# darchr/EmbeddingTables.jl

Measured on AMD Instinct MI355X. Metric: embedding lookups/sec + achieved HBM GB/s (% of roofline), 26 tables x dim128 at B=65536, higher is better.
Workload: dtype f32

## Files before the change

embeddingtables.jl_amd/csrc/et_lookup.hip:

```cpp
#include <type_traits>
#include "et_common.h"
#include "et_lookup_order.h"

#include <stdlib.h>
#include <string.h>

#include <mutex>
#include <utility>
#include <vector>

namespace et {

struct XcdQueue;
struct LookupPack {
    et_lookup_desc d[ET_MAX_TABLES_PER_LAUNCH];
    XcdQueue* queue = nullptr;
};

template <typename T, int D>
struct VecGeom {
    static constexpr int N = 16 / (int)sizeof(T);
    static constexpr int VPR = D / N;
    static constexpr int LPR = VPR < 64 ? VPR : 64;
    static constexpr int NV = VPR / LPR;
// ... 210 lines not shown
    const uint32_t ldt = (uint32_t)d.ld_table, nr = (uint32_t)d.nrows;
    const int vpr = MK ? d.dim / G::N : G::VPR;
    int64_t bag = chunk * per_round * rounds + wave * G::GPW + g;
    long long my_next = load_idx_chunk<G::LPR>(
        d.idx + (bag < batch ? bag : batch - 1) * d.ld_idx, cnt0, sub);
    for (int r = 0; r < rounds; ++r) {
        if (bag >= batch) break;
        const long long my = my_next;
        const int64_t nbag = bag + per_round;
        if (r + 1 < rounds)
            my_next = load_idx_chunk<G::LPR>(
                d.idx + (nbag < batch ? nbag : batch - 1) * d.ld_idx, cnt0, sub);
        bag_sum_vec<T, A, D, U, NT, NTL, PG, MK>(table, ldt, nr, (uint32_t)d.cols_per_page,
                                                 d.idx + bag * d.ld_idx, pool, my,
                                                 dst + bag * ld_dst + d.dst_row_off, g, sub, vpr);
        bag = nbag;
    }
}

typedef const __attribute__((address_space(4))) int64_t* cidx_ptr;

__device__ __forceinline__ cidx_ptr as_scalar_idx(const int64_t* p) {
    return (cidx_ptr)(uintptr_t)p;
}

__device__ __forceinline__ uint64_t row_off_s(int64_t v, uint32_t ldb, uint32_t nrows,
                                              uint32_t& bad) {
    const uint32_t lo = (uint32_t)v - 1u;
    const uint32_t borrow = (uint32_t)(((uint64_t)lo - (uint64_t)nrows) >> 32);
    bad |= (uint32_t)((uint64_t)v >> 32) | ~borrow;
    return (((uint64_t)__umulhi(lo, ldb)) << 32) | (uint64_t)(lo * ldb);
}

template <typename T, typename A, int UU, bool NTL>
__device__ __forceinline__ bool load_add_s(uintptr_t tb, uint32_t ldb, uint32_t nrows,
                                           cidx_ptr ia, cidx_ptr ib, uint64_t hmask,
                                           uint64_t lane_off, bool first_batch,
                                           A (&acc)[16 / sizeof(T)]) {
    constexpr int N = 16 / (int)sizeof(T);
    typedef const __attribute__((address_space(1))) u32x4 gvec;
    uint64_t oa[UU], dd[UU];
    uint32_t bad = 0u;
#pragma unroll
    for (int u = 0; u < UU; ++u) {
        oa[u] = row_off_s(ia[u], ldb, nrows, bad);
        dd[u] = row_off_s(ib[u], ldb, nrows, bad) - oa[u];
    }
    if (bad) return false;
    u32x4 buf[UU];
#pragma unroll
    for (int u = 0; u < UU; ++u) {
        const uint64_t a = ((dd[u] & hmask) + lane_off) + (tb + oa[u]);
        const gvec* src = reinterpret_cast<const gvec*>(a);
        if constexpr (NTL)
            buf[u] = __builtin_nontemporal_load(src);
        else
            buf[u] = *src;
    }
#pragma unroll
    for (int u = 0; u < UU; ++u) {
        T x[N];
        __builtin_memcpy(x, &buf[u], 16);
#pragma unroll
        for (int k = 0; k < N; ++k) {
            if (u == 0)
                acc[k] = first_batch ? A(x[k]) : A(acc[k] + A(x[k]));
            else
                acc[k] = A(acc[k] + A(x[k]));
        }
    }
    return true;
}

template <typename T, typename A>
__device__ __forceinline__ void bag_pair_checked(uintptr_t tb, uint32_t ldb, uint32_t nrows,
                                                 const int64_t* ia, const int64_t* ib, bool hi,
                                                 int sub, int pool, A* acc, int* bad) {
    constexpr int N = 16 / (int)sizeof(T);
    const int64_t* ip = hi ? ib : ia;
#pragma unroll 1
    for (int i = 0; i < pool; ++i) {
        const uint64_t r = (uint64_t)(ip[i] - 1);
        const bool ok = r < (uint64_t)nrows;
        *bad += ok ? 0 : 1;
        const u32x4 v = *(reinterpret_cast<const u32x4*>(
                              tb + (uint64_t)(ok ? (uint32_t)r : 0u) * ldb) + sub);
        T x[N];
        unpack16<T, N>(ok ? v : u32x4{0u, 0u, 0u, 0u}, x);
        for (int k = 0; k < N; ++k) acc[k] = i == 0 ? A(x[k]) : A(acc[k] + A(x[k]));
    }
}

template <typename T, typename A, int U, bool NT, bool NTL>
__device__ __forceinline__ void run_bags_s(const et_lookup_desc& d, int64_t batch,
                                           T* __restrict__ dst, int64_t ld_dst, int64_t chunk,
                                           int rounds) {
    constexpr int N = 16 / (int)sizeof(T);
    const int lane = threadIdx.x & 63;
    const int wave = __builtin_amdgcn_readfirstlane(threadIdx.x >> 6);
    const bool hi = lane >= 32;
    const int sub = lane & 31;
    uint32_t hm = hi ? ~0u : 0u;
    asm volatile("" : "+v"(hm));
    const uint64_t hmask = ((uint64_t)hm << 32) | hm, lane_off = (uint64_t)sub * 16u;
    const uintptr_t tb = reinterpret_cast<uintptr_t>(d.table);
    const uint32_t ldb = (uint32_t)(d.ld_table * (int64_t)sizeof(T)), nr = (uint32_t)d.nrows;
    const int pool = d.pool;
    int64_t bag = chunk * 8 * rounds + 2 * wave;
    for (int r = 0; r < rounds; ++r, bag += 8) {
        if (bag >= batch) break;
        const bool has_b = bag + 1 < batch;
        const cidx_ptr ia = as_scalar_idx(d.idx + bag * d.ld_idx);
        const cidx_ptr ib = has_b ? as_scalar_idx(d.idx + (bag + 1) * d.ld_idx) : ia;
        A acc[N];
#pragma unroll
        for (int k = 0; k < N; ++k) acc[k] = A(0);
        bool ok = true;
        int i0 = 0;
#define ET_LOAD_ADD_S(UU) \
    load_add_s<T, A, UU, NTL>(tb, ldb, nr, ia + i0, ib + i0, hmask, lane_off, i0 == 0, acc)
        for (; ok && i0 + U <= pool; i0 += U) ok = ET_LOAD_ADD_S(U);
        if constexpr (U > 4) {
            if (ok && pool - i0 >= 4) {
                ok = ET_LOAD_ADD_S(4);
                i0 += 4;
            }
        }
        if constexpr (U > 2) {
            if (ok && pool - i0 >= 2) {
                ok = ET_LOAD_ADD_S(2);
                i0 += 2;
            }
        }
        if (ok && pool - i0 >= 1) ok = ET_LOAD_ADD_S(1);
#undef ET_LOAD_ADD_S
        int bad = 0;
        if (!ok)
            bag_pair_checked<T, A>(tb, ldb, nr, d.idx + bag * d.ld_idx,
                                   d.idx + (has_b ? bag + 1 : bag) * d.ld_idx, hi, sub, pool, acc,
                                   &bad);
        if (hi && !has_b) bad = 0;
        if (bad && sub == 0) note_oob(bad);
        if (!hi || has_b) {
            T y[N];
#pragma unroll
            for (int k = 0; k < N; ++k) y[k] = T(acc[k]);
            u32x4* o =
                reinterpret_cast<u32x4*>(dst + (bag + (hi ? 1 : 0)) * ld_dst + d.dst_row_off) + sub;
            store16<NT>(o, pack16<T, N>(y));
        }
    }
}

template <typename T, typename A, int D, int U, bool NT, bool PG = false, bool MK = false,
          bool SG = false>
__global__ __launch_bounds__(256) void k_pooled_vec(LookupPack pack, int ntables, int64_t batch,
                                                    T* __restrict__ dst, int64_t ld_dst,
                                                    int rounds) {
    const int64_t item = blockIdx.x;
    const int t = (int)(item % ntables);
    const int64_t chunk = item / ntables;
    if constexpr (SG)
        run_bags_s<T, A, U, NT, false>(pack.d[t], batch, dst, ld_dst, chunk, rounds);
    else
        run_bags<T, A, D, U, NT, false, PG, MK>(pack.d[t], batch, dst, ld_dst, chunk, rounds);
}

constexpr int kXcds = 8;
static_assert(kXcds == et_order::kXcds && ET_MAX_TABLES_PER_LAUNCH == et_order::kMaxTables,
              "et_lookup_order.h");

constexpr int kMaxStripeEntries = et_order::kMaxEntries;
struct StripeMap {
    uint32_t entry[kXcds][kMaxStripeEntries];
    int nent;
    uint32_t ntload_mask;
    uint32_t prio_mask;
    int nheavy;
    int affinity;
    int fab_share;
    et_order::ClassOrder order[2];
};

template <typename T, typename A, int D, int U, bool NT, bool SG>
__device__ __forceinline__ void striped_body(const LookupPack& pack, const StripeMap& sm,
                                             int ntables, int64_t batch, T* __restrict__ dst,
                                             int64_t ld_dst, int rounds, int64_t stripe_chunks,
                                             int64_t nchunks, int x = blockIdx.x % kXcds,
                                             int64_t slot = blockIdx.x / kXcds) {
    const int k = (int)(slot % ntables);
    const int64_t j = slot / ntables;
    const uint32_t e = sm.entry[x][k];
    const int t = (int)(e & 0xff);
    const int64_t chunk = (int64_t)((e >> 8) & 0xff) * stripe_chunks + j;
    if (j >= stripe_chunks || chunk >= nchunks) return;
    if ((sm.prio_mask >> t) & 1u) __builtin_amdgcn_s_setprio(2);
    if constexpr (SG) {
        if ((sm.ntload_mask >> t) & 1u)
            run_bags_s<T, A, U, NT, true>(pack.d[t], batch, dst, ld_dst, chunk, rounds);
        else
            run_bags_s<T, A, U, NT, false>(pack.d[t], batch, dst, ld_dst, chunk, rounds);
    } else {
        if ((sm.ntload_mask >> t) & 1u)
            run_bags<T, A, D, U, NT, true>(pack.d[t], batch, dst, ld_dst, chunk, rounds);
        else
            run_bags<T, A, D, U, NT, false>(pack.d[t], batch, dst, ld_dst, chunk, rounds);
    }
}

#ifdef ET_WG_TIMELINE
constexpr uint32_t kTlCap = 1u << 17;
__device__ uint4 g_tl[kTlCap][2];
#endif

__device__ __forceinline__ uint64_t tl_begin() {
#ifdef ET_WG_TIMELINE
    return __builtin_amdgcn_s_memrealtime();
#else
    return 0;
#endif
}

__device__ __forceinline__ void tl_stamp(uint64_t t0, const StripeMap& sm, int ntables,
                                         int64_t stripe_chunks, int64_t nchunks, int x,
                                         int64_t slot) {
#ifdef ET_WG_TIMELINE
    __syncthreads();
    if (threadIdx.x == 0 && blockIdx.x < kTlCap) {
        const uint64_t t1 = __builtin_amdgcn_s_memrealtime();
        uint32_t xcc, hw;
        asm volatile("s_getreg_b32 %0, hwreg(HW_REG_XCC_ID)" : "=s"(xcc));
        asm volatile("s_getreg_b32 %0, hwreg(HW_REG_HW_ID)" : "=s"(hw));
        uint32_t t = 0xffu;
        if (x >= 0) {
            const int64_t j = slot / ntables;
            const uint32_t e = sm.entry[x][slot % ntables];
            const int64_t chunk = (int64_t)((e >> 8) & 0xff) * stripe_chunks + j;
            t = (j >= stripe_chunks || chunk >= nchunks ? 0xffu : (e & 0xffu)) | ((uint32_t)x << 8);
        }
        g_tl[blockIdx.x][0] = make_uint4((uint32_t)t0, (uint32_t)(t0 >> 32), (uint32_t)t1,
                                         (uint32_t)(t1 >> 32));
        g_tl[blockIdx.x][1] = make_uint4(t, xcc, hw, gridDim.x);
    }
#endif
}

template <typename T, typename A, int D, int U, bool NT, bool SG = false>
__global__ __launch_bounds__(256) void k_pooled_vec_striped(LookupPack pack, StripeMap sm,
                                                            int ntables, int64_t batch,
                                                            T* __restrict__ dst, int64_t ld_dst,
                                                            int rounds, int64_t stripe_chunks,
                                                            int64_t nchunks) {
    const uint64_t t0 = tl_begin();
    striped_body<T, A, D, U, NT, SG>(pack, sm, ntables, batch, dst, ld_dst, rounds, stripe_chunks,
                                     nchunks);
    tl_stamp(t0, sm, ntables, stripe_chunks, nchunks, blockIdx.x % kXcds, blockIdx.x / kXcds);
}

struct XcdQueue {
    uint32_t head[kXcds][2];
    uint32_t done;
    uint32_t pad[32 - 2 * kXcds - 1];
};
static_assert(sizeof(XcdQueue) == ET_LOOKUP_QUEUE_BYTES, "queue block size (include/embtab.h)");

__device__ __forceinline__ uint32_t cu_hash16(uint32_t hw) {
    const uint32_t cu = (hw >> 8) & 15u, sh = (hw >> 12) & 1u, se = (hw >> 13) & 7u;
    const uint32_t v = (cu + 3u * se + 5u * sh) & 15u;
    return ((v & 1u) << 3) | ((v & 2u) << 1) | ((v & 4u) >> 1) | ((v & 8u) >> 3);
}

__device__ __forceinline__ uint32_t claim_class(XcdQueue& q, const StripeMap& sm, uint32_t x,
                                                uint32_t c, uint32_t nheavy, uint32_t ntables,
                                                uint32_t sc) {
    const uint32_t h = atomicAdd(&q.head[x][c], 1u);
    const uint32_t slot = et_order::class_slot(sm.order[c], x, c, h, nheavy, ntables, sc);
    return slot == et_order::kNone ? ~0u : x * (ntables * sc) + slot;
}

__device__ __forceinline__ uint32_t claim_pref(XcdQueue& q, const StripeMap& sm, uint32_t x0,
                                               uint32_t p, uint32_t nheavy, uint32_t ntables,
                                               uint32_t sc) {
    constexpr uint32_t M = (uint32_t)(kXcds - 1);
    uint32_t it = claim_class(q, sm, x0, p, nheavy, ntables, sc);
    if (it == ~0u && p == 1u) it = claim_class(q, sm, x0, 0u, nheavy, ntables, sc);
    for (uint32_t k = 1; it == ~0u && k < (uint32_t)kXcds; ++k)
        it = claim_class(q, sm, (x0 + k) & M, 0u, nheavy, ntables, sc);
    if (it == ~0u && p == 0u) it = claim_class(q, sm, x0, 1u, nheavy, ntables, sc);
    for (uint32_t k = 1; it == ~0u && k < (uint32_t)kXcds; ++k)
        it = claim_class(q, sm, (x0 + k) & M, 1u, nheavy, ntables, sc);
    return it;
}

template <typename T, typename A, int D, int U, bool NT, bool SG>
__global__ __launch_bounds__(256) void k_pooled_vec_queued(LookupPack pack, StripeMap sm,
                                                           int ntables, int64_t batch,
                                                           T* __restrict__ dst, int64_t ld_dst,
                                                           int rounds, int64_t stripe_chunks,
                                                           int64_t nchunks) {
    const uint64_t t0 = tl_begin();
    __shared__ uint32_t s_item;
    XcdQueue& q = *pack.queue;
    const uint32_t per = (uint32_t)(ntables * stripe_chunks);
    if (threadIdx.x == 0) {
        uint32_t xcc;
        asm volatile("s_getreg_b32 %0, hwreg(HW_REG_XCC_ID)" : "=s"(xcc));
        uint32_t it = ~0u;
        if (sm.affinity != 0) {
            const uint32_t x0 = xcc & (uint32_t)(kXcds - 1);
            const uint32_t nh = (uint32_t)sm.nheavy, sc = (uint32_t)stripe_chunks;
            uint32_t hw;
            asm volatile("s_getreg_b32 %0, hwreg(HW_REG_HW_ID)" : "=s"(hw));
            const uint32_t p = cu_hash16(hw) < (uint32_t)sm.fab_share ? 0u : 1u;
            it = claim_pref(q, sm, x0, p, nh, (uint32_t)ntables, sc);
        } else
        for (uint32_t k = 0; k < (uint32_t)kXcds; ++k) {
            const uint32_t x = (xcc + k) & (uint32_t)(kXcds - 1);
            const uint32_t h = atomicAdd(&q.head[x][0], 1u);
            if (h < per) {
                it = x * per + h;
                break;
            }
        }
        s_item = it;
    }
    __syncthreads();
    const uint32_t it = s_item;
    if (it != ~0u)
        striped_body<T, A, D, U, NT, SG>(pack, sm, ntables, batch, dst, ld_dst, rounds,
                                         stripe_chunks, nchunks, (int)(it / per),
                                         (int64_t)(it % per));
    tl_stamp(t0, sm, ntables, stripe_chunks, nchunks, it != ~0u ? (int)(it / per) : -1,
             (int64_t)(it % per));
    if (threadIdx.x == 0 && atomicAdd(&q.done, 1u) == gridDim.x - 1u) {
        uint32_t* w = reinterpret_cast<uint32_t*>(&q);
        for (int i = 0; i < (int)(sizeof(XcdQueue) / sizeof(uint32_t)); ++i) atomicExch(&w[i], 0u);
    }
}

template <int RB, bool NT>
__global__ __launch_bounds__(256) void k_gather_vec(LookupPack pack, int ntables, int64_t batch,
                                                    char* __restrict__ dst, int64_t ld_dst_b,
                                                    int es, int rounds) {
    constexpr int VPR = RB / 16;
    constexpr int LPR = VPR < 64 ? VPR : 64;
    constexpr int NV = VPR / LPR;
// ... 44 lines not shown
                    store16<NT>(o + v * LPR, okv[u] ? buf[u][v] : u32x4{0u, 0u, 0u, 0u});
            }
        }
        if (bad && sub == 0) note_oob(bad);
    }
}

template <int RB, bool NT, bool NTL, int U, int W = 4>
__global__ __launch_bounds__(64 * W) void k_gather_one(LookupPack pack, int ntables, int64_t batch,
                                                       char* __restrict__ dst, int64_t ld_dst_b,
                                                       int es) {
#ifdef ET_WG_TIMELINE
    const uint64_t tl0 = __builtin_amdgcn_s_memrealtime();
#endif
    constexpr int VPR = RB / 16;
    static_assert(VPR <= 64 && 64 % VPR == 0, "one vector per lane");
    constexpr int GPW = 64 / VPR;
    const int64_t item = blockIdx.x;
    const int t = (int)(item % ntables);
    const int64_t chunk = item / ntables;
    const et_lookup_desc& d = pack.d[t];
    const char* table = reinterpret_cast<const char*>(d.table);
    const int64_t ld_b = d.ld_table * es;
    const int lane = threadIdx.x & 63, wave = threadIdx.x >> 6;
    const int g = lane / VPR, sub = lane % VPR;
    const int64_t per_round = W * GPW;
    const int64_t bag0 = chunk * per_round * U + wave * GPW + g;
    int64_t iv[U];
#pragma unroll
    for (int u = 0; u < U; ++u) {
        int64_t b = bag0 + u * per_round;
        b = b < batch ? b : batch - 1;
        iv[u] = d.idx[b * d.ld_idx];
    }
    u32x4 cur[U];
    bool ok[U];
#pragma unroll
    for (int u = 0; u < U; ++u) {
        const uint64_t row = (uint64_t)(iv[u] - 1);
        ok[u] = row < (uint64_t)d.nrows;
        const u32x4* src = reinterpret_cast<const u32x4*>(table + (ok[u] ? row * (uint64_t)ld_b : 0)) + sub;
        if constexpr (NTL) cur[u] = __builtin_nontemporal_load(src);
        else cur[u] = *src;
    }
#ifdef ET_WG_TIMELINE
    asm volatile("" ::: "memory");
    const uint64_t tl1 = __builtin_amdgcn_s_memrealtime();
#endif
    int bad = 0;
#pragma unroll
    for (int u = 0; u < U; ++u) {
        const int64_t bag = bag0 + u * per_round;
        if (bag < batch) {
            bad += ok[u] ? 0 : 1;
            u32x4* o = reinterpret_cast<u32x4*>(dst + bag * ld_dst_b + d.dst_row_off * es) + sub;
            store16<NT>(o, ok[u] ? cur[u] : u32x4{0u, 0u, 0u, 0u});
        }
    }
    if (bad && sub == 0) note_oob(bad);
#ifdef ET_WG_TIMELINE
    asm volatile("s_waitcnt vmcnt(0)" ::: "memory");
    __syncthreads();
    if (threadIdx.x == 0 && blockIdx.x < kTlCap) {
        const uint64_t tl2 = __builtin_amdgcn_s_memrealtime();
        uint32_t xcc;
        asm volatile("s_getreg_b32 %0, hwreg(HW_REG_XCC_ID)" : "=s"(xcc));
        g_tl[blockIdx.x][0] = make_uint4((uint32_t)tl0, (uint32_t)(tl0 >> 32), (uint32_t)tl1,
                                         (uint32_t)(tl1 >> 32));
        g_tl[blockIdx.x][1] = make_uint4((uint32_t)tl2, (uint32_t)(tl2 >> 32), xcc, gridDim.x);
    }
#endif
}

template <typename O, typename T>
__device__ __forceinline__ O convert_elt(T x) {
    if constexpr ((__is_same(T, __bf16) || __is_same(O, __bf16)) && !__is_same(T, float) &&
                  !__is_same(O, float))
        return O((float)x);
    else
        return O(x);
}

template <typename T, typename A, bool NT, typename O = T>
__global__ __launch_bounds__(256) void k_pooled_generic(LookupPack pack, int ntables,
                                                        int64_t batch, O* __restrict__ dst,
                                                        int64_t ld_dst) {
    constexpr int K = 4;
    const int64_t item = blockIdx.x;
    const int t = (int)(item % ntables);
    const int64_t chunk = item / ntables;
    const et_lookup_desc& d = pack.d[t];
    const T* table = reinterpret_cast<const T*>(d.table);
    const int lane = threadIdx.x & 63, wave = threadIdx.x >> 6;
    const int64_t bag = chunk * 4 + wave;
    if (bag >= batch) return;
    const int64_t* ip = d.idx + bag * d.ld_idx;
    O* out = dst + bag * ld_dst + d.dst_row_off;
    const int dim = d.dim, pool = d.pool;
    for (int f0 = 0; f0 < dim; f0 += 64 * K) {
        A acc[K];
#pragma unroll
        for (int k = 0; k < K; ++k) acc[k] = A(0);
        for (int i = 0; i < pool; ++i) {
            uint64_t row = (uint64_t)(ip[i] - 1);
            const bool ok = row < (uint64_t)d.nrows;
            if (!ok && lane == 0 && f0 == 0) note_oob();
            row = ok ? row : 0;
            const T* src = col_ptr<const T>(d.table, d.ld_table, d.cols_per_page, row);
#pragma unroll
            for (int k = 0; k < K; ++k) {
                const int f = f0 + lane + 64 * k;
                if (f < dim) {
                    const T x = ok ? src[f] : T(0);
                    acc[k] = i == 0 ? A(x) : A(acc[k] + A(x));
                }
            }
        }
#pragma unroll
        for (int k = 0; k < K; ++k) {
            const int f = f0 + lane + 64 * k;
            if (f < dim) store_scalar<NT>(out + f, convert_elt<O>(T(acc[k])));
        }
    }
}


inline bool gather_rb_ok(int64_t rb) {
    return rb == 32 || rb == 64 || rb == 128 || rb == 256 || rb == 512 || rb == 1024 ||
           rb == 2048 || rb == 4096;
}

int max_rounds();

inline int rounds_for(int64_t batch, int64_t bags_per_round, int ntables) {
    int64_t blocks1 = (batch + bags_per_round - 1) / bags_per_round * ntables;
    int rounds = 1;
    const int mr = max_rounds();
    while (rounds < mr && blocks1 / (rounds * 2) >= 4096) rounds *= 2;
    return rounds;
}

struct LookupTuning {
    int striped = 1;
    int queued = 1;
    int ntload = 1;
    int64_t ntload_bytes = 256ll << 20;
    int max_rounds = 8;
    int64_t light_bytes = 4 << 20;
    int sgpr = 1;
    int heavy_prio = 0;
    int affinity = 1;
    int fab_share = 8;
    et_order::Policy order = {1, 3, 1 << 20};
};

inline const LookupTuning& tuning() {
    static LookupTuning t = [] {
        LookupTuning v;
#ifdef ET_EXPERIMENTS
        if (const char* e = getenv("ET_SCHED")) {
            v.striped = strcmp(e, "linear") != 0;
            v.queued = v.striped && strcmp(e, "stripe") != 0;
        }
        v.ntload = (int)ET_KNOB("ET_NTLOAD", v.ntload);
        v.ntload_bytes = ET_KNOB("ET_NTLOAD_BYTES", v.ntload_bytes);
        v.max_rounds = (int)ET_KNOB("ET_ROUNDS", v.max_rounds);
        if (v.max_rounds < 1) v.max_rounds = 1;
        v.light_bytes = ET_KNOB("ET_LIGHT_BYTES", v.light_bytes);
        v.sgpr = (int)ET_KNOB("ET_SGPR", v.sgpr);
        v.heavy_prio = (int)ET_KNOB("ET_HEAVY_PRIO", v.heavy_prio);
        if (const char* e = getenv("ET_AFFINITY")) v.affinity = *e == 'A' ? 1 : 0;
        v.fab_share = (int)ET_KNOB("ET_FAB_SHARE", v.fab_share);
        v.order.cache_major = (int)ET_KNOB("ET_ORDER_CACHE", v.order.cache_major);
        v.order.fab = (int)ET_KNOB("ET_ORDER_FAB", v.order.fab);
        v.order.phase_bytes = ET_KNOB("ET_PHASE_BYTES", v.order.phase_bytes);
#endif
        return v;
    }();
    return t;
}

int max_rounds() { return tuning().max_rounds; }

inline void build_stripe_map(const LookupPack& pack, int n, int es, bool queued, StripeMap& sm) {
    const LookupTuning& tu = tuning();
    int64_t bytes[ET_MAX_TABLES_PER_LAUNCH];
    sm.ntload_mask = 0;
    sm.prio_mask = 0;
    for (int t = 0; t < n; ++t) {
        bytes[t] = pack.d[t].nrows * pack.d[t].ld_table * es;
        if (bytes[t] > tu.light_bytes) {
            if (tu.heavy_prio) sm.prio_mask |= 1u << t;
            if (tu.ntload && bytes[t] > tu.ntload_bytes) sm.ntload_mask |= 1u << t;
        }
    }
    sm.nent = et_order::place_stripes(bytes, n, tu.light_bytes, sm.entry, &sm.nheavy);
    sm.affinity = sm.nheavy > 0 && sm.nheavy < sm.nent ? tu.affinity : 0;
    sm.fab_share = tu.fab_share < 0 ? 0 : tu.fab_share > 16 ? 16 : tu.fab_share;
    if (sm.fab_share == 0) sm.affinity = 0;
    memset(sm.order, 0, sizeof(sm.order));
    if (queued && sm.affinity != 0)
        for (int x = 0; x < kXcds; ++x)
            et_order::order_xcd(sm.entry[x], x, sm.nent, sm.nheavy, bytes, sm.ntload_mask, tu.order,
                                sm.order);
}

template <typename T, typename A, int D, bool NT, bool PG = false, bool MK = false>
int launch_pooled_vec(const LookupPack& pack, int n, int64_t batch, void* dst, int64_t ld_dst,
                      hipStream_t s) {
    using G = VecGeom<T, D>;
    constexpr int U = G::U;
    constexpr bool kSG = !PG && !MK && D * (int)sizeof(T) == 512;
    bool sg = kSG && tuning().sgpr;
    for (int t = 0; t < n && sg; ++t) sg = pack.d[t].ld_table * (int64_t)sizeof(T) < (1ll << 32);
    const int64_t per_round = sg ? 8 : 4 * G::GPW;
    const int rounds = rounds_for(batch, per_round, n);
    const int64_t nchunks = (batch + per_round * rounds - 1) / (per_round * rounds);
    if (nchunks <= 0) return ET_OK;
    const bool striped = !PG && !MK && n > 1 && tuning().striped;
    StripeMap sm;
    int64_t stripe_chunks = 0, grid = nchunks * n;
    const bool queued = striped && pack.queue && tuning().queued;
    if (striped) {
        build_stripe_map(pack, n, (int)sizeof(T), queued, sm);
        stripe_chunks = (nchunks + kXcds - 1) / kXcds;
        grid = (int64_t)kXcds * sm.nent * stripe_chunks;
    }
    if (grid > 0x7fffffffll) return fail(ET_ERR_ARG, "grid too large");
    auto launch = [&](auto loop) -> int {
        constexpr bool SG = decltype(loop)::value;
        T* out = reinterpret_cast<T*>(dst);
        if constexpr (!PG && !MK) {
            if (queued) {
                hipLaunchKernelGGL((k_pooled_vec_queued<T, A, D, U, NT, SG>), dim3((unsigned)grid),
                                   dim3(256), 0, s, pack, sm, sm.nent, batch, out, ld_dst, rounds,
                                   stripe_chunks, nchunks);
                ET_LAUNCH_CHECK("k_pooled_vec_queued");
                return ET_OK;
            }
            if (striped) {
                hipLaunchKernelGGL((k_pooled_vec_striped<T, A, D, U, NT, SG>), dim3((unsigned)grid),
                                   dim3(256), 0, s, pack, sm, sm.nent, batch, out, ld_dst, rounds,
                                   stripe_chunks, nchunks);
                ET_LAUNCH_CHECK("k_pooled_vec_striped");
                return ET_OK;
            }
        }
        hipLaunchKernelGGL((k_pooled_vec<T, A, D, U, NT, PG, MK, SG>), dim3((unsigned)grid),
                           dim3(256), 0, s, pack, n, batch, out, ld_dst, rounds);
        ET_LAUNCH_CHECK("k_pooled_vec");
        return ET_OK;
    };
    if constexpr (kSG) {
        if (sg) return launch(std::true_type{});
    }
    return launch(std::false_type{});
}

template <int RB, bool NT>
int launch_gather_rb(const LookupPack& pack, int n, int64_t batch, void* dst, int64_t ld_dst,
                     int es, hipStream_t s) {
    constexpr int VPR = RB / 16;
    constexpr int LPR = VPR < 64 ? VPR : 64;
    constexpr int NV = VPR / LPR;
    constexpr int U = NV >= 8 ? 1 : 8 / NV;
    const int64_t per_round = 4 * (64 / LPR) * U;
    if constexpr (NV == 1 && U == 8) {
        bool ntl = tuning().ntload != 0;
        for (int t = 0; t < n && ntl; ++t)
            ntl = pack.d[t].nrows * pack.d[t].ld_table * es > tuning().ntload_bytes;
        constexpr int kU = 8, kW = 4;
        const int64_t pw = kW * (64 / LPR) * kU;
        const int64_t g1 = (batch + pw - 1) / pw * n;
        if (g1 <= 0) return ET_OK;
        if (g1 > 0x7fffffffll) return fail(ET_ERR_ARG, "grid too large");
        if (ntl)
            hipLaunchKernelGGL((k_gather_one<RB, NT, true, kU, kW>), dim3((unsigned)g1),
                               dim3(64 * kW), 0, s, pack, n, batch, reinterpret_cast<char*>(dst),
                               ld_dst * es, es);
        else
            hipLaunchKernelGGL((k_gather_one<RB, NT, false, kU, kW>), dim3((unsigned)g1),
                               dim3(64 * kW), 0, s, pack, n, batch, reinterpret_cast<char*>(dst),
                               ld_dst * es, es);
        ET_LAUNCH_CHECK("k_gather_one");
        return ET_OK;
    }
    const int rounds = rounds_for(batch, per_round, n);
    const int64_t nchunks = (batch + per_round * rounds - 1) / (per_round * rounds);
    const int64_t grid = nchunks * n;
    if (grid <= 0) return ET_OK;
    if (grid > 0x7fffffffll) return fail(ET_ERR_ARG, "grid too large");
    hipLaunchKernelGGL((k_gather_vec<RB, NT>), dim3((unsigned)grid), dim3(256), 0, s, pack, n,
                       batch, reinterpret_cast<char*>(dst), ld_dst * es, es, rounds);
    ET_LAUNCH_CHECK("k_gather_vec");
    return ET_OK;
}

template <bool NT>
int launch_gather(const LookupPack& pack, int n, int64_t rb, int64_t batch, void* dst,
                  int64_t ld_dst, int es, hipStream_t s) {
    switch (rb) {
        case 32: return launch_gather_rb<32, NT>(pack, n, batch, dst, ld_dst, es, s);
        case 64: return launch_gather_rb<64, NT>(pack, n, batch, dst, ld_dst, es, s);
        case 128: return launch_gather_rb<128, NT>(pack, n, batch, dst, ld_dst, es, s);
        case 256: return launch_gather_rb<256, NT>(pack, n, batch, dst, ld_dst, es, s);
        case 512: return launch_gather_rb<512, NT>(pack, n, batch, dst, ld_dst, es, s);
        case 1024: return launch_gather_rb<1024, NT>(pack, n, batch, dst, ld_dst, es, s);
        case 2048: return launch_gather_rb<2048, NT>(pack, n, batch, dst, ld_dst, es, s);
        case 4096: return launch_gather_rb<4096, NT>(pack, n, batch, dst, ld_dst, es, s);
    }
    return fail(ET_ERR_UNSUPPORTED, "gather row bytes %lld", (long long)rb);
}

template <typename T, typename A, bool NT, bool PG = false>
int launch_pooled_dim(const LookupPack& pack, int n, int D, int64_t batch, void* dst,
                      int64_t ld_dst, hipStream_t s) {
    switch (D) {
        case 16: return launch_pooled_vec<T, A, 16, NT, PG>(pack, n, batch, dst, ld_dst, s);
        case 32: return launch_pooled_vec<T, A, 32, NT, PG>(pack, n, batch, dst, ld_dst, s);
        case 64: return launch_pooled_vec<T, A, 64, NT, PG>(pack, n, batch, dst, ld_dst, s);
        case 128: return launch_pooled_vec<T, A, 128, NT, PG>(pack, n, batch, dst, ld_dst, s);
        case 256: return launch_pooled_vec<T, A, 256, NT, PG>(pack, n, batch, dst, ld_dst, s);
        case 512: return launch_pooled_vec<T, A, 512, NT, PG>(pack, n, batch, dst, ld_dst, s);
    }
    return fail(ET_ERR_UNSUPPORTED, "vector dim %d", D);
}

template <typename T, typename A, bool NT>
int launch_pooled_masked(const LookupPack& pack, int n, int D, int64_t batch, void* dst,
                         int64_t ld_dst, hipStream_t s) {
#define ET_MK(C)                                                                              \
    case C:                                                                                   \
        if constexpr (C / (16 / (int)sizeof(T)) >= 1)                                         \
            return launch_pooled_vec<T, A, C, NT, false, true>(pack, n, batch, dst, ld_dst,   \
                                                               s);                            \
        break;
    switch (masked_capacity(D)) {
        ET_MK(16)
        ET_MK(32)
        ET_MK(64)
        ET_MK(128)
        ET_MK(256)
        ET_MK(512)
        ET_MK(1024)
        ET_MK(2048)
    }
#undef ET_MK
    return fail(ET_ERR_UNSUPPORTED, "masked vector dim %d", D);
}

template <typename T, typename A, bool NT>
int launch_generic(const LookupPack& pack, int n, int64_t batch, void* dst, int64_t ld_dst,
                   hipStream_t s) {
    const int64_t grid = (batch + 3) / 4 * n;
    if (grid <= 0) return ET_OK;
    if (grid > 0x7fffffffll) return fail(ET_ERR_ARG, "grid too large");
    hipLaunchKernelGGL((k_pooled_generic<T, A, NT>), dim3((unsigned)grid), dim3(256), 0, s, pack,
                       n, batch, reinterpret_cast<T*>(dst), ld_dst);
    ET_LAUNCH_CHECK("k_pooled_generic");
    return ET_OK;
}

enum GroupKind { kGather = 0, kPooledVec = 1, kGeneric = 2, kPagedVec = 3, kMaskedVec = 4 };

template <typename T, typename A, bool NT>
int launch_group_typed(GroupKind kind, const LookupPack& pack, int n, int D, int64_t batch,
                       void* dst, int64_t ld_dst, hipStream_t s) {
    const int es = (int)sizeof(T);
    if (kind == kGather)
        return launch_gather<NT>(pack, n, (int64_t)D * es, batch, dst, ld_dst, es, s);
    if (kind == kPooledVec) return launch_pooled_dim<T, A, NT>(pack, n, D, batch, dst, ld_dst, s);
    if (kind == kPagedVec)
        return launch_pooled_dim<T, A, NT, true>(pack, n, D, batch, dst, ld_dst, s);
    if (kind == kMaskedVec)
        return launch_pooled_masked<T, A, NT>(pack, n, D, batch, dst, ld_dst, s);
    return launch_generic<T, A, NT>(pack, n, batch, dst, ld_dst, s);
}
// ... 297 lines not shown
```

embeddingtables.jl_amd/csrc/et_lookup_order.h:

```cpp
#pragma once
#include <stdint.h>

#if defined(__HIPCC__) || defined(__CUDACC__)
#define ET_ORDER_FN __host__ __device__ inline
#else
#define ET_ORDER_FN inline
#endif

namespace et_order {

constexpr int kXcds = 8;
constexpr uint32_t kNone = ~0u;
constexpr uint32_t kTablesFastest = 0, kTableMajor = 1;

struct ClassOrder {
    uint8_t split[kXcds];
    uint8_t major[kXcds];
};

ET_ORDER_FN uint32_t class_slot(uint32_t h, uint32_t nk, uint32_t base, uint32_t ntables,
                                uint32_t sc, uint32_t split, uint32_t major0, uint32_t major1) {
    if (h >= nk * sc) return kNone;
    if (split > nk) split = nk;
    uint32_t n = split, first = 0, major = major0;
    if (h >= split * sc) {
        h -= split * sc;
        n = nk - split;
        first = split;
        major = major1;
    }
    const uint32_t j = major == kTableMajor ? h % sc : h / n;
    const uint32_t k = major == kTableMajor ? h / sc : h % n;
    return j * ntables + base + first + k;
}

ET_ORDER_FN uint32_t class_slot(const ClassOrder& o, uint32_t x, uint32_t c, uint32_t h,
                                uint32_t nheavy, uint32_t ntables, uint32_t sc) {
    const uint32_t nk = c ? ntables - nheavy : nheavy;
    return class_slot(h, nk, c ? nheavy : 0u, ntables, sc, o.split[x], o.major[x] & 1u,
                      (o.major[x] >> 1) & 1u);
}


constexpr int kMaxEntries = 40;
constexpr int kMaxTables = 32;

inline uint32_t entry_table(uint32_t e) { return e & 0xffu; }

inline int place_stripes(const int64_t* table_bytes, int n, int64_t light_bytes,
                         uint32_t entry[][kMaxEntries], int* nheavy) {
    int heavy[kMaxTables], light[kMaxTables];
    int nh = 0, nl = 0;
    for (int t = 0; t < n; ++t)
        if (table_bytes[t] > light_bytes) heavy[nh++] = t;
        else light[nl++] = t;
    for (int a = 0; a < nl; ++a)
        for (int b = a + 1; b < nl; ++b)
            if (table_bytes[light[b]] > table_bytes[light[a]]) {
                int tmp = light[a];
                light[a] = light[b];
                light[b] = tmp;
            }
    int order[kMaxTables];
    for (int i = 0, lo = 0, hi = nl - 1; i < nl; ++i) order[i] = (i & 1) ? light[hi--] : light[lo++];
    int cnt[kXcds] = {0};
    for (int x = 0; x < kXcds; ++x)
        for (int h = 0; h < nh; ++h) entry[x][cnt[x]++] = (uint32_t)heavy[h] | ((uint32_t)x << 8);
    for (int q = 0; q < nl * kXcds; ++q) {
        const int x = q / (nl > 0 ? nl : 1);
        entry[x][cnt[x]++] = (uint32_t)order[q / kXcds] | ((uint32_t)(q % kXcds) << 8);
    }
    *nheavy = nh;
    return cnt[0];
}


template <typename F>
inline int stable_front(uint32_t* e, int n, F first) {
    uint32_t tmp[256];
    int a = 0, b = 0;
    for (int i = 0; i < n; ++i)
        if (first(e[i])) e[a++] = e[i];
        else tmp[b++] = e[i];
    for (int i = 0; i < b; ++i) e[a + i] = tmp[i];
    return a;
}

inline void rotate_left(uint32_t* e, int n, int r) {
    if (n <= 1) return;
    uint32_t tmp[256];
    for (int i = 0; i < n; ++i) tmp[i] = e[(i + r) % n];
    for (int i = 0; i < n; ++i) e[i] = tmp[i];
}

inline void largest_first(uint32_t* e, int n, const int64_t* table_bytes) {
    for (int i = 1; i < n; ++i) {
        const uint32_t v = e[i];
        int k = i;
        for (; k > 0 && table_bytes[entry_table(e[k - 1])] < table_bytes[entry_table(v)]; --k)
            e[k] = e[k - 1];
        e[k] = v;
    }
}

inline int64_t class_footprint(const uint32_t* e, int n, const int64_t* table_bytes) {
    uint32_t seen = 0;
    int64_t sum = 0;
    for (int i = 0; i < n; ++i) {
        const uint32_t t = entry_table(e[i]);
        if (!((seen >> t) & 1u)) sum += table_bytes[t];
        seen |= 1u << t;
    }
    return sum;
}

inline int two_phases(uint32_t* e, int n, uint32_t nt_mask, bool nt_first, int rot) {
    const int nnt =
        stable_front(e, n, [&](uint32_t v) { return ((nt_mask >> entry_table(v)) & 1u) != 0; });
    const int nal = n - nnt;
    if (nal > 0) rotate_left(e + nnt, nal, rot % nal);
    if (nt_first) return nnt;
    rotate_left(e, n, nnt);
    return nal;
}

struct Policy {
    int cache_major = 0;
    int fab = 0;
    int64_t phase_bytes = 1 << 20;
};

inline void order_xcd(uint32_t* e, int x, int ntables, int nheavy, const int64_t* table_bytes,
                      uint32_t nt_mask, const Policy& p, ClassOrder ord[2]) {
    uint32_t* ce = e + nheavy;
    const int nc = ntables - nheavy;
    ord[0].split[x] = ord[1].split[x] = 0;
    ord[0].major[x] = ord[1].major[x] = 0;
    if (p.cache_major) {
        largest_first(ce, nc, table_bytes);
        ord[1].major[x] = 3;
    }
    if (p.fab == 1 || p.fab == 2) {
        const bool nt_first = class_footprint(ce, nc, table_bytes) > p.phase_bytes;
        ord[0].split[x] = (uint8_t)two_phases(e, nheavy, nt_mask, nt_first, p.fab == 2 ? x : 0);
        if (p.fab == 2) ord[0].major[x] = nt_first ? 2 : 1;
    } else if (p.fab == 3) {
        rotate_left(e, nheavy, nheavy > 0 ? x % nheavy : 0);
        ord[0].major[x] = 3;
    }
}

}
```

Measured before the change: 29.51 billion.

## Split mid-size tables into column quarters striped across XCDs for cache locality

Tables between 4 and 16 MB are split by column into four quarters, and each XCD handles one quarter for half the batch. The per-XCD working set of such a table therefore shrinks to a quarter, so it can stay resident in that XCD's cache. A new quarter-width gather loop (8 lanes per row, 32 bags per round) and new stripe-map encoding bits support the split, and the fabric share default changes when quartering is active. The cost is more work items and narrower 128-byte row segments per gather, which may lower per-request efficiency.

```diff
diff --git a/embeddingtables.jl_amd/csrc/et_lookup.hip b/embeddingtables.jl_amd/csrc/et_lookup.hip
--- a/embeddingtables.jl_amd/csrc/et_lookup.hip
+++ b/embeddingtables.jl_amd/csrc/et_lookup.hip
@@ -386,6 +386,108 @@
     }
 }
 
+template <typename T, typename A, int UU>
+__device__ __forceinline__ void load_add_q(const char* __restrict__ tb, uint32_t myoff, int gaddr,
+                                           uint32_t lane_off, int i0, bool first_batch,
+                                           bool anybad, A (&acc)[16 / sizeof(T)], int& bad) {
+    constexpr int N = 16 / (int)sizeof(T);
+    uint32_t off[UU];
+#pragma unroll
+    for (int u = 0; u < UU; ++u)
+        off[u] = (uint32_t)__builtin_amdgcn_ds_bpermute(gaddr + 4 * (i0 + u), (int)myoff);
+    u32x4 buf[UU];
+    if (__builtin_expect(anybad, 0)) {
+#pragma unroll
+        for (int u = 0; u < UU; ++u) {
+            const bool ok = off[u] != ~0u;
+            bad += ok ? 0 : 1;
+            const u32x4 v = *reinterpret_cast<const u32x4*>(tb + ((ok ? off[u] : 0u) + lane_off));
+            buf[u] = ok ? v : u32x4{0u, 0u, 0u, 0u};
+        }
+    } else {
+#pragma unroll
+        for (int u = 0; u < UU; ++u)
+            buf[u] = *reinterpret_cast<const u32x4*>(tb + (off[u] + lane_off));
+    }
+#pragma unroll
+    for (int u = 0; u < UU; ++u) {
+        T x[N];
+        unpack16<T, N>(buf[u], x);
+#pragma unroll
+        for (int k = 0; k < N; ++k) {
+            if (u == 0)
+                acc[k] = first_batch ? A(x[k]) : A(acc[k] + A(x[k]));
+            else
+                acc[k] = A(acc[k] + A(x[k]));
+        }
+    }
+}
+
+template <typename T, typename A, int U, bool NT>
+__device__ __forceinline__ void run_bags_q(const et_lookup_desc& d, int64_t batch,
+                                           T* __restrict__ dst, int64_t ld_dst, int64_t chunk,
+                                           int rounds, bool count_bad) {
+    constexpr int N = 16 / (int)sizeof(T), LPR = 8, GPW = 8;
+    static_assert(U == 2 || U == 4 || U == 8, "rows in flight of the quarter loop");
+    const int lane = threadIdx.x & 63, wave = threadIdx.x >> 6;
+    const int g = lane / LPR, sub = lane % LPR;
+    const int gaddr = (g * LPR) << 2;
+    const uint32_t lane_off = (uint32_t)sub * 16u;
+    const char* tb = reinterpret_cast<const char*>(d.table);
+    const uint32_t ldb = (uint32_t)(d.ld_table * (int64_t)sizeof(T)), nr = (uint32_t)d.nrows;
+    const int pool = d.pool;
+    const int cnt0 = pool < LPR ? pool : LPR;
+    const int64_t per_round = 4 * GPW;
+    int64_t bag = chunk * per_round * rounds + wave * GPW + g;
+    long long my_next =
+        load_idx_chunk<LPR>(d.idx + (bag < batch ? bag : batch - 1) * d.ld_idx, cnt0, sub);
+    for (int r = 0; r < rounds; ++r) {
+        if (bag >= batch) break;
+        long long my = my_next;
+        const int64_t nbag = bag + per_round;
+        if (r + 1 < rounds)
+            my_next = load_idx_chunk<LPR>(
+                d.idx + (nbag < batch ? nbag : batch - 1) * d.ld_idx, cnt0, sub);
+        const int64_t* ip = d.idx + bag * d.ld_idx;
+        A acc[N];
+#pragma unroll
+        for (int k = 0; k < N; ++k) acc[k] = A(0);
+        int bad = 0;
+        for (int c0 = 0; c0 < pool; c0 += LPR) {
+            const int cnt = pool - c0 < LPR ? pool - c0 : LPR;
+            if (c0 != 0) my = load_idx_chunk<LPR>(ip + c0, cnt, sub);
+            const uint32_t row = idx_row32(my, nr);
+            const uint32_t myoff = row == ~0u ? ~0u : row * ldb;
+            const bool anybad = __any(row == ~0u) != 0;
+            int i0 = 0;
+#define ET_LOAD_ADD_Q(UU) \
+    load_add_q<T, A, UU>(tb, myoff, gaddr, lane_off, i0, c0 + i0 == 0, anybad, acc, bad)
+            for (; i0 + U <= cnt; i0 += U) ET_LOAD_ADD_Q(U);
+            if constexpr (U > 4) {
+                if (cnt - i0 >= 4) {
+                    ET_LOAD_ADD_Q(4);
+                    i0 += 4;
+                }
+            }
+            if constexpr (U > 2) {
+                if (cnt - i0 >= 2) {
+                    ET_LOAD_ADD_Q(2);
+                    i0 += 2;
+                }
+            }
+            if (cnt - i0 >= 1) ET_LOAD_ADD_Q(1);
+#undef ET_LOAD_ADD_Q
+        }
+        if (bad && sub == 0 && count_bad) note_oob(bad);
+        T y[N];
+#pragma unroll
+        for (int k = 0; k < N; ++k) y[k] = T(acc[k]);
+        store16<NT>(reinterpret_cast<u32x4*>(dst + bag * ld_dst + d.dst_row_off) + sub,
+                    pack16<T, N>(y));
+        bag = nbag;
+    }
+}
+
 template <typename T, typename A, int D, int U, bool NT, bool PG = false, bool MK = false,
           bool SG = false>
 __global__ __launch_bounds__(256) void k_pooled_vec(LookupPack pack, int ntables, int64_t batch,
@@ -404,6 +506,10 @@
 static_assert(kXcds == et_order::kXcds && ET_MAX_TABLES_PER_LAUNCH == et_order::kMaxTables,
               "et_lookup_order.h");
 
+#ifndef ET_QUARTER_U
+#define ET_QUARTER_U 4
+#endif
+constexpr int kQuarterU = ET_QUARTER_U;
 constexpr int kMaxStripeEntries = et_order::kMaxEntries;
 struct StripeMap {
     uint32_t entry[kXcds][kMaxStripeEntries];
@@ -426,6 +532,22 @@
     const int64_t j = slot / ntables;
     const uint32_t e = sm.entry[x][k];
     const int t = (int)(e & 0xff);
+    if constexpr (SG) {
+        if (et_order::entry_quartered(e)) {
+            constexpr int DQ = D / 4;
+            static_assert(4 * VecGeom<T, DQ>::GPW == et_order::kQuarterBagsPerRound, "");
+            const et_order::ItemBags ib =
+                et_order::item_bags(e, j, stripe_chunks, nchunks, rounds, batch);
+            if (ib.count == 0) return;
+            const int q = (int)et_order::entry_quarter(e);
+            et_lookup_desc dq = pack.d[t];
+            dq.table = reinterpret_cast<const T*>(dq.table) + q * DQ;
+            dq.dst_row_off += q * DQ;
+            if ((sm.prio_mask >> t) & 1u) __builtin_amdgcn_s_setprio(2);
+            run_bags_q<T, A, kQuarterU, NT>(dq, batch, dst, ld_dst, ib.chunk, rounds, q == 0);
+            return;
+        }
+    }
     const int64_t chunk = (int64_t)((e >> 8) & 0xff) * stripe_chunks + j;
     if (j >= stripe_chunks || chunk >= nchunks) return;
     if ((sm.prio_mask >> t) & 1u) __builtin_amdgcn_s_setprio(2);
@@ -776,6 +898,10 @@
     int affinity = 1;
     int fab_share = 8;
     et_order::Policy order = {1, 3, 1 << 20};
+    int64_t quarter_min_bytes = 4 << 20;
+    int64_t quarter_max_bytes = 16 << 20;
+    int quarter_cache = 1;
+    int quarter_fab_share = 7;
 };
 
 inline const LookupTuning& tuning() {
@@ -798,6 +924,10 @@
         v.order.cache_major = (int)ET_KNOB("ET_ORDER_CACHE", v.order.cache_major);
         v.order.fab = (int)ET_KNOB("ET_ORDER_FAB", v.order.fab);
         v.order.phase_bytes = ET_KNOB("ET_PHASE_BYTES", v.order.phase_bytes);
+        v.quarter_min_bytes = ET_KNOB("ET_QUARTER_MIN", v.quarter_min_bytes);
+        v.quarter_max_bytes = ET_KNOB("ET_QUARTER_MAX", v.quarter_max_bytes);
+        if (const char* e = getenv("ET_QUARTER_CLASS")) v.quarter_cache = strcmp(e, "cache") == 0;
+        v.quarter_fab_share = (int)ET_KNOB("ET_FAB_SHARE", v.quarter_fab_share);
 #endif
         return v;
     }();
@@ -806,26 +936,36 @@
 
 int max_rounds() { return tuning().max_rounds; }
 
-inline void build_stripe_map(const LookupPack& pack, int n, int es, bool queued, StripeMap& sm) {
+inline void build_stripe_map(const LookupPack& pack, int n, int es, bool queued, bool sg,
+                             StripeMap& sm) {
     const LookupTuning& tu = tuning();
-    int64_t bytes[ET_MAX_TABLES_PER_LAUNCH];
+    int64_t bytes[ET_MAX_TABLES_PER_LAUNCH], foot[ET_MAX_TABLES_PER_LAUNCH];
+    uint32_t quarter_mask = 0;
     sm.ntload_mask = 0;
     sm.prio_mask = 0;
     for (int t = 0; t < n; ++t) {
         bytes[t] = pack.d[t].nrows * pack.d[t].ld_table * es;
+        foot[t] = bytes[t];
+        if (sg && pack.d[t].ld_table == pack.d[t].dim && bytes[t] > tu.quarter_min_bytes &&
+            bytes[t] <= tu.quarter_max_bytes && bytes[t] < (1ll << 31)) {
+            quarter_mask |= 1u << t;
+            foot[t] = bytes[t] / 4;
+        }
         if (bytes[t] > tu.light_bytes) {
             if (tu.heavy_prio) sm.prio_mask |= 1u << t;
             if (tu.ntload && bytes[t] > tu.ntload_bytes) sm.ntload_mask |= 1u << t;
         }
     }
-    sm.nent = et_order::place_stripes(bytes, n, tu.light_bytes, sm.entry, &sm.nheavy);
+    sm.nent = et_order::place_stripes(bytes, n, tu.light_bytes, quarter_mask, tu.quarter_cache != 0,
+                                      sm.entry, &sm.nheavy);
     sm.affinity = sm.nheavy > 0 && sm.nheavy < sm.nent ? tu.affinity : 0;
-    sm.fab_share = tu.fab_share < 0 ? 0 : tu.fab_share > 16 ? 16 : tu.fab_share;
+    const int share = quarter_mask != 0 && tu.quarter_cache ? tu.quarter_fab_share : tu.fab_share;
+    sm.fab_share = share < 0 ? 0 : share > 16 ? 16 : share;
     if (sm.fab_share == 0) sm.affinity = 0;
     memset(sm.order, 0, sizeof(sm.order));
     if (queued && sm.affinity != 0)
         for (int x = 0; x < kXcds; ++x)
-            et_order::order_xcd(sm.entry[x], x, sm.nent, sm.nheavy, bytes, sm.ntload_mask, tu.order,
+            et_order::order_xcd(sm.entry[x], x, sm.nent, sm.nheavy, foot, sm.ntload_mask, tu.order,
                                 sm.order);
 }
 
@@ -846,7 +986,7 @@
     int64_t stripe_chunks = 0, grid = nchunks * n;
     const bool queued = striped && pack.queue && tuning().queued;
     if (striped) {
-        build_stripe_map(pack, n, (int)sizeof(T), queued, sm);
+        build_stripe_map(pack, n, (int)sizeof(T), queued, sg, sm);
         stripe_chunks = (nchunks + kXcds - 1) / kXcds;
         grid = (int64_t)kXcds * sm.nent * stripe_chunks;
     }
diff --git a/embeddingtables.jl_amd/csrc/et_lookup_order.h b/embeddingtables.jl_amd/csrc/et_lookup_order.h
--- a/embeddingtables.jl_amd/csrc/et_lookup_order.h
+++ b/embeddingtables.jl_amd/csrc/et_lookup_order.h
@@ -42,18 +42,48 @@
 }
 
 
+constexpr uint32_t kQuarterFlag = 1u << 18;
+
+ET_ORDER_FN uint32_t entry_table(uint32_t e) { return e & 0xffu; }
+ET_ORDER_FN uint32_t entry_stripe(uint32_t e) { return (e >> 8) & 0xffu; }
+ET_ORDER_FN uint32_t entry_quarter(uint32_t e) { return (e >> 16) & 3u; }
+ET_ORDER_FN bool entry_quartered(uint32_t e) { return (e & kQuarterFlag) != 0; }
+
+constexpr int kRowBagsPerRound = 8, kQuarterBagsPerRound = 32;
+
+struct ItemBags {
+    int64_t chunk, first, count;
+};
+ET_ORDER_FN ItemBags item_bags(uint32_t e, int64_t j, int64_t sc, int64_t nchunks, int64_t rounds,
+                               int64_t batch) {
+    ItemBags b;
+    b.chunk = (int64_t)entry_stripe(e) * sc + j;
+    const int64_t per = (entry_quartered(e) ? kQuarterBagsPerRound : kRowBagsPerRound) * rounds;
+    b.first = b.chunk * per;
+    b.count = 0;
+    if (j >= sc || b.first >= batch) return b;
+    if (!entry_quartered(e) && b.chunk >= nchunks) return b;
+    b.count = batch - b.first < per ? batch - b.first : per;
+    return b;
+}
+
+
 constexpr int kMaxEntries = 40;
 constexpr int kMaxTables = 32;
 
-inline uint32_t entry_table(uint32_t e) { return e & 0xffu; }
-
 inline int place_stripes(const int64_t* table_bytes, int n, int64_t light_bytes,
+                         uint32_t quarter_mask, bool quarter_cache,
                          uint32_t entry[][kMaxEntries], int* nheavy) {
-    int heavy[kMaxTables], light[kMaxTables];
-    int nh = 0, nl = 0;
+    int heavy[kMaxTables], light[kMaxTables], qcache[kMaxTables];
+    int nh = 0, nl = 0, nq = 0;
+    auto quartered = [&](int t) { return ((quarter_mask >> t) & 1u) != 0; };
     for (int t = 0; t < n; ++t)
-        if (table_bytes[t] > light_bytes) heavy[nh++] = t;
+        if (quartered(t) && quarter_cache) qcache[nq++] = t;
+        else if (quartered(t) || table_bytes[t] > light_bytes) heavy[nh++] = t;
         else light[nl++] = t;
+    auto quarter_entry = [](int t, int x) {
+        return (uint32_t)t | ((uint32_t)(x / 4) << 8) | ((uint32_t)(x % 4) << 16) | kQuarterFlag;
+    };
     for (int a = 0; a < nl; ++a)
         for (int b = a + 1; b < nl; ++b)
             if (table_bytes[light[b]] > table_bytes[light[a]]) {
@@ -64,8 +94,12 @@
     int order[kMaxTables];
     for (int i = 0, lo = 0, hi = nl - 1; i < nl; ++i) order[i] = (i & 1) ? light[hi--] : light[lo++];
     int cnt[kXcds] = {0};
-    for (int x = 0; x < kXcds; ++x)
-        for (int h = 0; h < nh; ++h) entry[x][cnt[x]++] = (uint32_t)heavy[h] | ((uint32_t)x << 8);
+    for (int x = 0; x < kXcds; ++x) {
+        for (int h = 0; h < nh; ++h)
+            entry[x][cnt[x]++] = quartered(heavy[h]) ? quarter_entry(heavy[h], x)
+                                                     : (uint32_t)heavy[h] | ((uint32_t)x << 8);
+        for (int h = 0; h < nq; ++h) entry[x][cnt[x]++] = quarter_entry(qcache[h], x);
+    }
     for (int q = 0; q < nl * kXcds; ++q) {
         const int x = q / (nl > 0 ? nl : 1);
         entry[x][cnt[x]++] = (uint32_t)order[q / kXcds] | ((uint32_t)(q % kXcds) << 8);
@@ -74,6 +108,10 @@
     return cnt[0];
 }
 
+inline int place_stripes(const int64_t* table_bytes, int n, int64_t light_bytes,
+                         uint32_t entry[][kMaxEntries], int* nheavy) {
+    return place_stripes(table_bytes, n, light_bytes, 0u, false, entry, nheavy);
+}
 
 template <typename F>
 inline int stable_front(uint32_t* e, int n, F first) {
```

After: 30.71 billion, median of 6. 4.0% higher.
